# eric070021/TFHE-GPU

Measured on AMD Instinct MI355X. Metric: bootstraps/sec (whole node), STD128 GINX global batch=8192 (8192 per GPU, weak scaling), higher is better.
Workload: dtype u32; 1 GPU; C2: STD128 GINX EvalBinGate(NAND), inputs resident in HBM; config=C2, global_batch=8192, batch_per_gpu=8192, bootstraps_per_unit=1, n=512, N=1024, Q=134215681, dG2=8, parallelism=shard1

## Files before the change

tfhe-gpu_amd/csrc/blind_rotate_fast.hip:

```cpp
#include <atomic>
#include <cstdlib>

#include "device_math.hpp"
#include "kernels.hpp"

namespace tfhe {
namespace {

constexpr uint32_t FN = 1024;
constexpr uint32_t T4W = 5416, TB_WORDS = T4W;

struct FastConst {
    int32_t Q, nQ, qinv, rM;
    uint32_t Q2, Q4, h1, kacc;
    int32_t ninv;
    uint32_t bm;
};

struct PackMode {
    uint32_t hc[8];
    uint32_t rw;
    uint32_t fold;
};
__global__ void k_pack_fast(uint32_t Q, const uint32_t* __restrict__ bsk, size_t words, int32_t* __restrict__ out,
                            PackMode M) {
    const size_t idx = (size_t)blockIdx.x * blockDim.x + threadIdx.x;
    auto mont = [Q](uint32_t v) {
        const uint32_t m = (uint32_t)(((uint64_t)v << 32) % Q);
        return m > Q / 2 ? (int32_t)m - (int32_t)Q : (int32_t)m;
    };
    if (idx < words) {
        const uint32_t row = (uint32_t)((idx / (2 * FN)) % M.rw), l = row >> 1, p = row & 1, top = M.rw / 2 - 1;
        uint32_t v = bsk[idx] % Q;
// ... 10 lines not shown

static Fast4Shape fast_shape(const BRParams& P) {
    Fast4Shape sh{(int)P.digits, (int)P.logG, (int)P.thr, false};
    if (P.thr == 0 && P.digits >= 2 && P.logG >= 1 && P.logG * P.digits <= 40) {
        const int64_t G = (int64_t)1 << P.logG, Qh = (int64_t)(P.Q >> 1);
        const uint32_t top = P.digits - 1;
        int64_t K = 0;
        for (uint32_t z = 0; z < top; ++z) K = K * G + G / 2;
        const int64_t lo = (-Qh - 1 + K) >> (P.logG * top), hi = (Qh - 1 + K) >> (P.logG * top);
        sh.fold = lo >= -G / 2 && hi < G / 2;
    }
    return sh;
}

bool fast_path_supported(const BRParams& P, int word_bits) {
    return word_bits == 32 && P.N == FN && P.dG2 == 2 * P.digits && P.Q < (1ull << 27) && P.n > 0 &&
           fast4_shape_supported(fast_shape(P));
}

size_t bsk_fast_bytes(const BRParams& P) { return ((size_t)P.n * 2 * P.dG2 * 2 * FN + TB_WORDS) * 4; }

namespace {
constexpr int kDefaultVariant = 60;
bool known_variant(int v) { return v == 60 || v == 70 || v == 86; }
std::atomic<int> g_variant{-1};
int fast_variant() {
    int v = g_variant.load(std::memory_order_relaxed);
    if (v < 0) {
        const char* e = std::getenv("TFHE_FAST_VARIANT");
        v = e && e[0] ? std::atoi(e) : kDefaultVariant;
        if (!known_variant(v)) v = kDefaultVariant;
        g_variant.store(v, std::memory_order_relaxed);
    }
    return v;
}
uint64_t powmod(uint64_t b, uint64_t e, uint64_t m) {
    uint64_t r = 1 % m;
    for (b %= m; e; e >>= 1, b = (unsigned __int128)b * b % m)
        if (e & 1) r = (unsigned __int128)r * b % m;
    return r;
}
int32_t mont_centred(uint64_t v, uint32_t Q) {
    const uint32_t m = (uint32_t)(((unsigned __int128)(v % Q) << 32) % Q);
    return m > Q / 2 ? (int32_t)m - (int32_t)Q : (int32_t)m;
}
}

// ... 61 lines not shown
```

tfhe-gpu_amd/csrc/blind_rotate_fast4.hip:

```cpp
#include "device_math.hpp"
#include "kernels.hpp"

namespace tfhe {
namespace f4 {

constexpr uint32_t FN = 1024;
constexpr int TPC = 256;

constexpr uint32_t P0F = 0, P1F = 4, P2F = 20, P3F = 84, P4F = 340, PF_END = 1364;
constexpr uint32_t P0I = PF_END, P1I = P0I + P1F, P4I = P0I + P4F;
constexpr uint32_t T4_MONO = 2 * PF_END, T4_T1 = T4_MONO + 2 * FN, T4_T23 = T4_T1 + 128, T4_T2131 = T4_T23 + 256,
                   T4_WORDS = T4_T2131 + 256;
constexpr uint32_t L_TW = 0, L_TWI = P4F - P1F, L_MONO = 2 * L_TWI;
constexpr uint32_t L_T1 = L_MONO + 2 * FN, L_T23 = L_T1 + 128, L_T2131 = L_T23 + 256, L_P4F = L_T2131 + 256;
constexpr uint32_t LP = 304, XP = 1152, L_CT = L_P4F + 4 * 256;
constexpr uint32_t lds_ct(bool P4 = true) { return P4 ? L_CT : L_P4F; }
constexpr size_t lds_bytes(int P, int XB = 2, int CTS = 1, bool P4 = true) {
    return (size_t)(lds_ct(P4) + CTS * (4 * P * LP + XB * P * XP)) * 4;
}
constexpr bool pair_build(int MINW, int NCT, int OPT) { return MINW == 3 && NCT == 2 && (OPT & 8) == 0; }

struct Lay {
    int reg[2];
    int lane[6];
    int wave[2];
};
__host__ __device__ constexpr Lay lay(int L) {
    return L == 1   ? Lay{{8, 9}, {2, 3, 4, 6, 7, 5}, {0, 1}}
           : L == 2 ? Lay{{6, 7}, {2, 3, 8, 9, 4, 5}, {0, 1}}
           : L == 3 ? Lay{{4, 5}, {2, 3, 6, 8, 9, 7}, {0, 1}}
           : L == 4 ? Lay{{2, 3}, {4, 5, 6, 8, 9, 7}, {0, 1}}
                    : Lay{{0, 1}, {2, 3, 4, 5, 6, 7}, {8, 9}};
}
__host__ __device__ constexpr int rstride(int A, int B) {
    return (A == 1 && B == 2) ? 72 : (A == 2 && B == 3) ? 80 : (A == 3 && B == 4) ? 65
         : (A == 2 && B == 1) ? 68 : (A == 3 && B == 2) ? 68 : (A == 4 && B == 3) ? 65
// ... 75 lines not shown
__device__ __forceinline__ void bfly_ct(int32_t& a, int32_t& b, int32_t w, const FastConst& K) {
    const int32_t v = smul(b, w, K), u = a;
    a = u + v;
    b = u - v;
}
template <bool RED = false>
__device__ __forceinline__ void bfly_gs(int32_t& a, int32_t& b, int32_t w, const FastConst& K) {
    const int32_t u = a, v = b;
    a = RED ? smul(u + v, K.rM, K) : u + v;
    b = smul(u - v, w, K);
}
__device__ __forceinline__ void fwd4(int32_t (&x)[4], int32_t w1, int32_t w2, int32_t w3, const FastConst& K) {
    bfly_ct(x[0], x[2], w1, K);
    bfly_ct(x[1], x[3], w1, K);
    bfly_ct(x[0], x[1], w2, K);
    bfly_ct(x[2], x[3], w3, K);
}
template <bool RED>
__device__ __forceinline__ void inv4(int32_t (&x)[4], int32_t w1, int32_t w2, int32_t w3, const FastConst& K) {
    bfly_gs(x[0], x[1], w2, K);
    bfly_gs(x[2], x[3], w3, K);
    bfly_gs<RED>(x[0], x[2], w1, K);
    bfly_gs<RED>(x[1], x[3], w1, K);
}

template <int A, int B, uint32_t OFF>
__device__ __forceinline__ void store_rows(const int32_t (&x)[4], uint32_t m0, const int32_t* lds) {
    asm volatile(
        "s_mov_b32 m0, %4\n\t"
        "s_nop 0\n\t"
        "ds_write_addtid_b32 %0 offset:%6\n\t"
        "ds_write_addtid_b32 %1 offset:%7\n\t"
        "ds_write_addtid_b32 %2 offset:%8\n\t"
        "ds_write_addtid_b32 %3 offset:%9" ::"v"(x[0]),
        "v"(x[1]), "v"(x[2]), "v"(x[3]), "s"(m0), "s"(lds), "i"((OFF + st_reg(A, B, 0)) * 4),
        "i"((OFF + st_reg(A, B, 1)) * 4), "i"((OFF + st_reg(A, B, 2)) * 4), "i"((OFF + st_reg(A, B, 3)) * 4)
        : "memory");
}
template <int A, int B, uint32_t OFF>
__device__ __forceinline__ void gather_rows(int32_t (&x)[4], uint32_t base, const int32_t* lds) {
    asm volatile(
        "ds_read_b32 %0, %4 offset:%6\n\t"
        "ds_read_b32 %1, %4 offset:%7\n\t"
        "ds_read_b32 %2, %4 offset:%8\n\t"
        "ds_read_b32 %3, %4 offset:%9"
        : "=&v"(x[0]), "=&v"(x[1]), "=&v"(x[2]), "=&v"(x[3])
        : "v"(base), "s"(lds), "i"((OFF + ld_reg(A, B, 0)) * 4), "i"((OFF + ld_reg(A, B, 1)) * 4),
          "i"((OFF + ld_reg(A, B, 2)) * 4), "i"((OFF + ld_reg(A, B, 3)) * 4)
        : "memory");
}
template <uint32_t OFF>
__device__ __forceinline__ void tw_load(v4i& w, uint32_t addr, const int32_t* lds) {
    asm volatile("ds_read_b128 %0, %1 offset:%3" : "=&v"(w) : "v"(addr), "s"(lds), "i"(OFF * 4) : "memory");
}
template <int N>
__device__ __forceinline__ void lds_wait(int32_t (&x)[4]) {
    asm volatile("s_waitcnt lgkmcnt(%4)" : "+v"(x[0]), "+v"(x[1]), "+v"(x[2]), "+v"(x[3]) : "i"(N) : "memory");
}
template <int N>
__device__ __forceinline__ void lds_wait(int32_t (&x)[4], v4i& w) {
    asm volatile("s_waitcnt lgkmcnt(%5)"
                 : "+v"(x[0]), "+v"(x[1]), "+v"(x[2]), "+v"(x[3]), "+v"(w)
                 : "i"(N)
                 : "memory");
}
__device__ __forceinline__ void lds_drain_barrier() {
    asm volatile("s_waitcnt lgkmcnt(0)" ::: "memory");
    __syncthreads();
}

struct LaneCtx {
    uint32_t g12, g23, g34, g45, g54, g43, g32, g21;
    uint32_t m_loc;
    uint32_t m45, m54;
    uint32_t t1, t2, t3, t4;
    int32_t w0f[3], w0i[3];
    v4i w4f, w4i;
};

#define FOR_P(...)                                   \
    {                                                \
        { constexpr int p = 0; __VA_ARGS__ }         \
        if constexpr (P > 1) {                       \
            { constexpr int p = 1; __VA_ARGS__ }     \
        }                                            \
        if constexpr (P > 2) {                       \
            { constexpr int p = 2; __VA_ARGS__ }     \
            { constexpr int p = 3; __VA_ARGS__ }     \
        }                                            \
    }
template <int P, int p>
constexpr int tail_wait() { return 4 * (P - 1 - p); }

template <uint32_t XA, int P, int EXP = 0, int SMALL = 0, bool PRE = false, bool P4L = false>
__device__ __forceinline__ void ntt_fwd(int32_t (&X)[P][4], const int32_t* lds, const LaneCtx& C, const FastConst& K) {
    if constexpr ((EXP & 8) != 0) return;
    constexpr int W = 4 * (P - 1);
    v4i w;
    if constexpr (SMALL == 2) {
        const int32_t* t1 = lds + L_T1 + 64;
        const int2* t23 = reinterpret_cast<const int2*>(lds + L_T23) + 64;
        const int2* t2131 = reinterpret_cast<const int2*>(lds + L_T2131) + 64;
        int32_t a[P];
        int2 u23[P], u2131[P];
        FOR_P(a[p] = t1[X[p][2]]; u23[p] = t23[X[p][1]]; u2131[p] = t2131[X[p][3]];)
        FOR_P(const int32_t x0 = X[p][0], u = u23[p].x + u2131[p].x, v = u23[p].y - u2131[p].y;
              const int32_t e0 = x0 + a[p], e2 = x0 - a[p];
              X[p][0] = e0 + u; X[p][1] = e0 - u; X[p][2] = e2 + v; X[p][3] = e2 - v;
              store_rows<1, 2, p * LP>(X[p], C.m_loc, lds);)
    } else if constexpr (SMALL == 1) {
        const int32_t* t1 = lds + L_T1 + 64;
        int32_t v[P][2];
        FOR_P(v[p][0] = t1[X[p][2]]; v[p][1] = t1[X[p][3]];)
        FOR_P(const int32_t a0 = X[p][0], a1 = X[p][1];
              X[p][0] = a0 + v[p][0]; X[p][2] = a0 - v[p][0]; X[p][1] = a1 + v[p][1]; X[p][3] = a1 - v[p][1];
              bfly_ct(X[p][0], X[p][1], C.w0f[1], K); bfly_ct(X[p][2], X[p][3], C.w0f[2], K);
              store_rows<1, 2, p * LP>(X[p], C.m_loc, lds);)
    } else {
        FOR_P(fwd4(X[p], C.w0f[0], C.w0f[1], C.w0f[2], K); store_rows<1, 2, p * LP>(X[p], C.m_loc, lds);)
    }
    tw_load<L_TW>(w, C.t1, lds);
    FOR_P(gather_rows<1, 2, p * LP>(X[p], C.g12, lds);)
    FOR_P(if constexpr (p == 0) lds_wait<W>(X[0], w); else lds_wait<W>(X[p]);
          fwd4(X[p], w.x, w.y, w.z, K); store_rows<2, 3, p * LP>(X[p], C.m_loc, lds);)
    tw_load<L_TW + 16>(w, C.t2, lds);
    FOR_P(gather_rows<2, 3, p * LP>(X[p], C.g23, lds);)
    FOR_P(if constexpr (p == 0) lds_wait<W>(X[0], w); else lds_wait<W>(X[p]);
          fwd4(X[p], w.x, w.y, w.z, K); store_rows<3, 4, p * LP>(X[p], C.m_loc, lds);)
    tw_load<L_TW + 80>(w, C.t3, lds);
    FOR_P(gather_rows<3, 4, p * LP>(X[p], C.g34, lds);)
    FOR_P(if constexpr (p == 0) lds_wait<W>(X[0], w); else lds_wait<W>(X[p]);
          fwd4(X[p], w.x, w.y, w.z, K);
          if constexpr (PRE && p == 0) __builtin_amdgcn_s_barrier();
          store_rows<4, 5, XA + p * XP>(X[p], C.m45, lds);)
    if constexpr (!(EXP & 1)) lds_drain_barrier();
    if constexpr (P4L) tw_load<L_P4F>(w, C.t4, lds);
    FOR_P(gather_rows<4, 5, XA + p * XP>(X[p], C.g45, lds);)
    if constexpr (P4L) {
        FOR_P(if constexpr (p == 0) lds_wait<tail_wait<P, 0>()>(X[0], w); else lds_wait<tail_wait<P, p>()>(X[p]);
              fwd4(X[p], w.x, w.y, w.z, K);)
    } else {
        FOR_P(lds_wait<tail_wait<P, p>()>(X[p]); fwd4(X[p], C.w4f.x, C.w4f.y, C.w4f.z, K);)
    }
}

template <uint32_t XA, int P, int EXP = 0, bool PRE = false>
__device__ __forceinline__ void ntt_inv(int32_t (&X)[P][4], const int32_t* lds, const LaneCtx& C, const FastConst& K) {
    if constexpr ((EXP & 8) != 0) return;
    constexpr int W = 4 * (P - 1);
    v4i w;
    FOR_P(inv4<false>(X[p], C.w4i.x, C.w4i.y, C.w4i.z, K); if constexpr (PRE && p == 0) __builtin_amdgcn_s_barrier();
          store_rows<5, 4, XA + p * XP>(X[p], C.m54, lds);)
    if constexpr (!(EXP & 1)) lds_drain_barrier();
    tw_load<L_TWI + 80>(w, C.t3, lds);
    FOR_P(gather_rows<5, 4, XA + p * XP>(X[p], C.g54, lds);)
    FOR_P(if constexpr (p == 0) lds_wait<W>(X[0], w); else lds_wait<W>(X[p]);
          inv4<true>(X[p], w.x, w.y, w.z, K);
          store_rows<4, 3, p * LP>(X[p], C.m_loc, lds);)
    tw_load<L_TWI + 16>(w, C.t2, lds);
    FOR_P(gather_rows<4, 3, p * LP>(X[p], C.g43, lds);)
    FOR_P(if constexpr (p == 0) lds_wait<W>(X[0], w); else lds_wait<W>(X[p]);
          inv4<false>(X[p], w.x, w.y, w.z, K); store_rows<3, 2, p * LP>(X[p], C.m_loc, lds);)
    tw_load<L_TWI>(w, C.t1, lds);
    FOR_P(gather_rows<3, 2, p * LP>(X[p], C.g32, lds);)
    FOR_P(if constexpr (p == 0) lds_wait<W>(X[0], w); else lds_wait<W>(X[p]);
          inv4<true>(X[p], w.x, w.y, w.z, K); store_rows<2, 1, p * LP>(X[p], C.m_loc, lds);)
    FOR_P(gather_rows<2, 1, p * LP>(X[p], C.g21, lds);)
    FOR_P(lds_wait<tail_wait<P, p>()>(X[p]); inv4<false>(X[p], C.w0i[0], C.w0i[1], C.w0i[2], K);)
}

template <int MINW, int NCT = 1, int EXP = 0, int OPT = 7, int XB = 2, int CTS = 1, int DIG = 4, int LOGG = 7,
          int THR = 0, bool FOLD = true, bool FLAG = false, bool SPLIT = false, int RING = 4>
__global__ void __launch_bounds__(TPC * (SPLIT ? 2 : CTS), MINW)
k_blind_rotate_fast4(FastConst K, uint32_t n, uint32_t loga, const int32_t* __restrict__ tabs,
                     const int32_t* __restrict__ bsk, const uint64_t* __restrict__ a, uint64_t* __restrict__ acc_io,
                     uint32_t B, uint32_t* __restrict__ done) {
    constexpr int NPOL = SPLIT ? 1 : 2;
    constexpr int P = NPOL * NCT;
    constexpr int GR = SPLIT ? 2 : CTS;
    extern __shared__ __align__(16) int32_t lds[];
    static_assert(CTS == 1 || NCT == 1, "CTS > 1 needs NCT = 1");
    static_assert(RING == 4 || RING == 2, "key ring of four groups or two");
    constexpr uint32_t LCT = lds_ct(!pair_build(MINW, NCT, OPT));
    static_assert(!SPLIT || (NCT == 1 && CTS == 1 && FOLD && !FLAG && XB == 1), "SPLIT: the folded one-ciphertext build");
    constexpr uint32_t RW = 2 * DIG;
    constexpr int TOP = DIG - 1;
    constexpr int NT = FOLD ? DIG - 1 : DIG;
    static_assert(!FOLD || THR == 0, "top-digit elimination needs every digit");
    static_assert(LOGG * (THR + NT) <= 32, "digit field beyond 32 bits");
    static_assert(XB == 1 || (DIG == 4 && FOLD), "two cross areas need the STD128 digit order");
    const uint32_t cl = __builtin_amdgcn_readfirstlane(threadIdx.x / TPC);
    const uint32_t tid = threadIdx.x % TPC;
    const uint32_t wg_ct = SPLIT ? blockIdx.x : blockIdx.x * CTS * NCT + cl;
    const uint32_t pol = SPLIT ? cl : 0;
    for (uint32_t k = threadIdx.x; k < L_TWI; k += TPC * GR) lds[L_TW + k] = tabs[P1F + k], lds[L_TWI + k] = tabs[P1I + k];
    for (uint32_t k = threadIdx.x; k < 2 * FN + 640; k += TPC * GR) lds[L_MONO + k] = tabs[T4_MONO + k];
    if constexpr ((OPT & 8) != 0)
        for (uint32_t k = threadIdx.x; k < 4 * 256; k += TPC * GR) lds[L_P4F + k] = tabs[P4F + k];
    const uint32_t w = __builtin_amdgcn_readfirstlane(tid >> 6), lane = tid & 63;
    constexpr uint32_t LOCW = P * LP, XAW = P * XP;
    constexpr uint32_t XA0 = 4 * LOCW, XA1 = XB == 2 ? XA0 + XAW : XA0;
    constexpr bool PRE = XB == 1;

    LaneCtx C;
    constexpr uint32_t CTW = 4 * LOCW + XB * XAW;
    const uint32_t ctb = (LCT + cl * CTW) * 4;
    C.m_loc = ctb + w * LOCW * 4;
    C.g12 = C.m_loc + ld_lane<1, 2>(w, lane) * 4, C.g23 = C.m_loc + ld_lane<2, 3>(w, lane) * 4;
    C.g34 = C.m_loc + ld_lane<3, 4>(w, lane) * 4, C.g43 = C.m_loc + ld_lane<4, 3>(w, lane) * 4;
    C.g32 = C.m_loc + ld_lane<3, 2>(w, lane) * 4, C.g21 = C.m_loc + ld_lane<2, 1>(w, lane) * 4;
    C.g45 = ctb + ld_lane<4, 5>(w, lane) * 4, C.g54 = ctb + ld_lane<5, 4>(w, lane) * 4;
    C.m45 = ctb + st_wave<4, 5>(w) * 4, C.m54 = ctb + st_wave<5, 4>(w) * 4;
    C.t1 = (elem<2>(w, lane, 0) >> 8) * 16, C.t2 = (elem<3>(w, lane, 0) >> 6) * 16;
    C.t3 = (elem<4>(w, lane, 0) >> 4) * 16, C.t4 = tid * 16;
    const v4i* tv = reinterpret_cast<const v4i*>(tabs);
    if constexpr ((OPT & 8) == 0) C.w4f = tv[P4F / 4 + tid];
    C.w4i = tv[P4I / 4 + tid];
#pragma unroll
    for (int k = 0; k < 3; ++k) C.w0f[k] = tabs[P0F + k], C.w0i[k] = tabs[P0I + k];

    const uint32_t Qh = (uint32_t)K.Q >> 1;
    int32_t acc[NCT][NPOL][4];
#pragma unroll
    for (int q = 0; q < NCT; ++q) {
        const uint32_t ct = wg_ct + q;
        const uint64_t* g = acc_io + (size_t)(ct < B ? ct : 0) * 2 * FN;
#pragma unroll
        for (int p = 0; p < NPOL; ++p)
#pragma unroll
            for (int r = 0; r < 4; ++r) {
                const uint64_t v0 = ct < B ? g[(SPLIT ? pol : p) * FN + elem<1>(w, lane, r)] : 0;
                const uint32_t v = (uint32_t)(v0 >= (uint64_t)K.Q ? v0 % (uint64_t)K.Q : v0);
                acc[q][p][r] = v < Qh ? (int32_t)v : (int32_t)v - K.Q;
            }
    }
    __syncthreads();

    int32_t Cp[P][4];
    if constexpr (FOLD) {
        if constexpr (SPLIT) {
#pragma unroll
            for (int r = 0; r < 4; ++r) Cp[0][r] = acc[0][0][r];
        } else {
#pragma unroll
            for (int q = 0; q < NCT; ++q)
#pragma unroll
                for (int r = 0; r < 4; ++r) Cp[2 * q][r] = acc[q][0][r], Cp[2 * q + 1][r] = acc[q][NPOL - 1][r];
        }
        ntt_fwd<XA1, P, EXP, 0, PRE, (OPT & 8) != 0>(Cp, lds, C, K);
#pragma unroll
        for (int p = 0; p < P; ++p)
#pragma unroll
            for (int r = 0; r < 4; ++r) Cp[p][r] = smul(Cp[p][r], K.ninv, K);
    }

    constexpr uint32_t ROWB = 2 * RW * 2 * FN * 4;
    const __amdgpu_buffer_rsrc_t rsrc =
        __builtin_amdgcn_make_buffer_rsrc(const_cast<int32_t*>(bsk), 0, (int)(n * ROWB), 0x00020000);
    const uint32_t voff = tid * 16;
    const uint32_t et = 2 * (__builtin_bitreverse32(tid) >> 24) + 1;
    const uint32_t amask = (1u << loga) - 1, ashift = 11 - loga;

    auto issue = [&](v4i (&pw)[2], uint32_t round_off, int l, int gi) {
        const int k = gi >> 1, j = gi & 1;
        if constexpr ((EXP & 2) != 0) {
            pw[0] = v4i{(int)round_off, l, gi, 4}, pw[1] = pw[0] + 1;
            return;
        }
        if constexpr (SPLIT) {
            pw[0] = ld_bsk(rsrc, voff, round_off + ((k * RW + 2 * l + pol) * 2 + j) * FN * 4);
            return;
        }
        pw[0] = ld_bsk(rsrc, voff, round_off + ((k * RW + 2 * l) * 2 + j) * FN * 4);
        pw[1] = ld_bsk(rsrc, voff, round_off + ((k * RW + 2 * l + 1) * 2 + j) * FN * 4);
    };
    auto mac = [&](int64_t (&s)[NCT][2][2][4], const int32_t (&X)[P][4], const v4i (&pw)[2], int gi, bool first) {
        const int k = gi >> 1, j = gi & 1;
        const int32_t w0[4] = {pw[0].x, pw[0].y, pw[0].z, pw[0].w};
        const int32_t w1[4] = {pw[1].x, pw[1].y, pw[1].z, pw[1].w};
#pragma unroll
        for (int q = 0; q < NCT; ++q)
#pragma unroll
            for (int r = 0; r < 4; ++r) {
// ... 42 lines not shown
        } else {
#pragma unroll
            for (int gi = 0; gi < RING; ++gi) issue(pw[gi], round_off, 0, gi);
        }
#pragma unroll
        for (uint32_t l = 0; l < NT; ++l) {
            const uint32_t lt = l + THR;
            const int32_t kl = (int32_t)(((1u << (LOGG * lt)) - 1) / ((1u << LOGG) - 1)) << (LOGG - 1);
            int32_t X[P][4];
            if constexpr (SPLIT) {
#pragma unroll
                for (int r = 0; r < 4; ++r) X[0][r] = __builtin_amdgcn_sbfe(acc[0][0][r] + kl, LOGG * lt, LOGG);
            } else {
#pragma unroll
                for (int q = 0; q < NCT; ++q)
#pragma unroll
                    for (int r = 0; r < 4; ++r) {
                        X[2 * q][r] = __builtin_amdgcn_sbfe(acc[q][0][r] + kl, LOGG * lt, LOGG);
                        X[2 * q + 1][r] = __builtin_amdgcn_sbfe(acc[q][NPOL - 1][r] + kl, LOGG * lt, LOGG);
                    }
            }
            __builtin_amdgcn_sched_barrier(0);
            constexpr int SM = LOGG > 7 ? 0 : (OPT & 4) ? 2 : (OPT & 1) ? 1 : 0;
            if (l & 1) ntt_fwd<XA1, P, EXP, SM, PRE, (OPT & 8) != 0>(X, lds, C, K);
            else ntt_fwd<XA0, P, EXP, SM, PRE, (OPT & 8) != 0>(X, lds, C, K);
            const bool last = l + 1 == NT;
            const uint32_t noff = !last ? round_off : (i + 1 < n ? i + 1 : i) * ROWB;
            const int nl = !last ? (int)l + 1 : TOP;
#pragma unroll
            for (int gi = 0; gi < 4; ++gi) {
                __builtin_amdgcn_sched_barrier(0);
                mac(s, X, pw[gi % RING], gi, !FOLD && l == 0);
                if constexpr (RING == 4) {
                    if (FOLD || !last) issue(pw[gi], noff, nl, gi);
                } else {
                    step2(round_off, (int)l, noff, nl, gi, !last);
                }
            }
        }

        __builtin_amdgcn_sched_barrier(0);
        const char* mono = reinterpret_cast<const char*>(lds + L_MONO);
        int32_t S[P][4];
        if constexpr (SPLIT) {
            int32_t* xch = lds + LCT + GR * (4 * P * LP + XB * P * XP);
            const uint32_t bp = (et * ai[0]) & 2047, bn = (0u - bp) & 2047;
            const uint32_t F4p = ((bp >> 4) & 0x1C) | ((bp & 63) << 7), F4n = ((bn >> 4) & 0x1C) | ((bn & 63) << 7);
            const uint32_t hp = (bp >> 4) & 0x60, hn = (bn >> 4) & 0x60;
            int32_t Am[2][4];
#pragma unroll
            for (int k = 0; k < 2; ++k)
#pragma unroll
                for (int r = 0; r < 4; ++r) {
                    xch[((pol * 2 + k) * 4 + r) * TPC + tid] = sredc(pol ? s[0][k][0][r] : s[0][k][1][r], K);
                    Am[k][r] = sredc(pol ? s[0][k][1][r] : s[0][k][0][r], K);
                }
            __syncthreads();
#pragma unroll
            for (int r = 0; r < 4; ++r) {
                const uint32_t c = ((r & 1) << 1) | (r >> 1);
                const uint32_t cs = c * 32 * ai[0];
                const int32_t mp = *reinterpret_cast<const int32_t*>(mono + ((((hp + cs) & 0x60)) | F4p));
                const int32_t mn = *reinterpret_cast<const int32_t*>(mono + ((((hn - cs) & 0x60)) | F4n));
                const int32_t A0 = Am[0][r] + xch[(((1 - pol) * 2 + 0) * 4 + r) * TPC + tid];
// ... 16 lines not shown
                const int32_t A10 = sredc(s[q][1][0][r], K), A11 = sredc(s[q][1][1][r], K);
                S[2 * q][r] = sredc((int64_t)A00 * mp + (int64_t)A10 * mn, K);
                S[2 * q + 1][r] = sredc((int64_t)A01 * mp + (int64_t)A11 * mn, K);
            }
        }
        if constexpr (FOLD) {
#pragma unroll
            for (int p = 0; p < P; ++p)
#pragma unroll
                for (int r = 0; r < 4; ++r) Cp[p][r] += S[p][r];
        }
        if (FOLD && (i & 7) == 7) {
#pragma unroll
            for (int p = 0; p < P; ++p)
#pragma unroll
                for (int r = 0; r < 4; ++r) Cp[p][r] = smul(Cp[p][r], K.rM, K);
        }
        __builtin_amdgcn_sched_barrier(0);
        if constexpr (FOLD && RING == 2) {
            const uint32_t noff = (i + 1 < n ? i + 1 : i) * ROWB;
            issue(pw[0], noff, TOP, 0), issue(pw[1], noff, TOP, 1);
            __builtin_amdgcn_sched_barrier(0);
        }
        ntt_inv<XA1, P, EXP, PRE>(S, lds, C, K);
#pragma unroll
        for (int q = 0; q < NCT; ++q)
#pragma unroll
            for (int p = 0; p < NPOL; ++p)
#pragma unroll
                for (int r = 0; r < 4; ++r) {
                    uint32_t u = (uint32_t)(acc[q][p][r] + S[NPOL * q + p][r]) + K.kacc;
                    if constexpr ((OPT & 2) != 0) {
                        const uint32_t qt = __umulhi(u, K.bm);
                        uint64_t t;
                        asm("v_mad_u64_u32 %0, vcc, %1, %2, %3" : "=v"(t) : "v"(qt), "s"(K.nQ), "v"((uint64_t)u) : "vcc");
                        u = csub32((uint32_t)t, (uint32_t)K.Q);
                    } else {
                        u = csub32(csub32(csub32(u, K.Q4), K.Q2), (uint32_t)K.Q);
                    }
                    acc[q][p][r] = (int32_t)(u - K.h1);
                }
    }
#pragma unroll
    for (int q = 0; q < NCT; ++q) {
        const uint32_t ct = wg_ct + q;
        if (ct >= B) continue;
        uint64_t* g = acc_io + (size_t)ct * 2 * FN;
// ... 31 lines not shown
        if (idx < P1F) m = 1, base = P0F;
        else if (idx < P2F) m = 4, base = P1F;
        else if (idx < P3F) m = 16, base = P2F;
        else if (idx < P4F) m = 64, base = P3F;
        else m = 256, base = P4F;
        const uint32_t c = (idx - base) >> 2, e = (idx - base) & 3;
        const uint32_t k = e == 0 ? m + c : 2 * m + 2 * c + (e - 1);
        out[idx] = e == 3 ? 0 : mont(psi[k]);
        out[P0I + idx] = e == 3 ? 0 : mont(ipsi[k]);
    }
    if (idx < 2 * FN) out[T4_MONO + ((idx >> 6) | ((idx & 63) << 5))] = mont(mono[idx]);
    if (idx < 128) {
        const int32_t d = (int32_t)idx - 64;
        auto dmul = [Q, d](uint64_t w) {
            const uint32_t v = (uint32_t)((uint64_t)(uint32_t)(d < 0 ? -d : d) * (w % Q) % Q);
            const uint32_t m = d < 0 ? (v ? Q - v : 0) : v;
            return m > Q / 2 ? (int32_t)m - (int32_t)Q : (int32_t)m;
        };
        const uint64_t p21 = (uint64_t)psi[2] * psi[1] % Q, p31 = (uint64_t)psi[3] * psi[1] % Q;
        out[T4_T1 + idx] = dmul(psi[1]);
        out[T4_T23 + 2 * idx] = dmul(psi[2]), out[T4_T23 + 2 * idx + 1] = dmul(psi[3]);
        out[T4_T2131 + 2 * idx] = dmul(p21), out[T4_T2131 + 2 * idx + 1] = dmul(p31);
    }
}

#endif
}
#ifndef TFHE_FAST4_KERNEL_ONLY

size_t fast4_table_words() { return f4::T4_WORDS; }
size_t fast4_lds_bytes(bool pair) { return pair ? f4::lds_bytes(4, 1, 1, false) : f4::lds_bytes(2, 1, 1); }

hipError_t launch_pack_tables_fast4(uint32_t Q, const DevTables& T, void* out, hipStream_t s) {
    hipLaunchKernelGGL(f4::k_pack_tables4, dim3((f4::T4_WORDS + 255) / 256), dim3(256), 0, s, Q,
                       (const uint32_t*)T.psi, (const uint32_t*)T.ipsi, (const uint32_t*)T.mono, (int32_t*)out);
    return hipGetLastError();
}

bool fast4_shape_supported(const Fast4Shape& sh) {
    return (sh.dig == 4 && sh.logg == 7 && sh.thr == 0 && sh.fold) ||
           (sh.dig == 6 && sh.logg == 5 && sh.thr == 0 && sh.fold) ||
           (sh.dig == 5 && sh.logg == 5 && sh.thr == 1 && !sh.fold) ||
           (sh.dig == 3 && sh.logg == 9 && sh.thr == 0 && !sh.fold);
}

hipError_t launch_blind_rotate_fast4_d6(const f4::FastConst& K, uint32_t n, uint32_t loga, const int32_t* tabs4,
                                        const int32_t* bsk, const uint64_t* a, uint64_t* acc, size_t B, hipStream_t s);

hipError_t launch_blind_rotate_fast4_pair(const f4::FastConst& K, uint32_t n, uint32_t loga, const int32_t* tabs4,
                                          const int32_t* bsk, const uint64_t* a, uint64_t* acc, size_t B, hipStream_t s);

hipError_t launch_blind_rotate_fast4(int variant, const Fast4Shape& sh, const void* K, uint32_t n, uint32_t loga,
                                     const int32_t* tabs4, const int32_t* bsk, const uint64_t* a, uint64_t* acc,
                                     size_t B, hipStream_t s, BRDone* dn, int split_max, int pair_min, bool* paired) {
    const f4::FastConst Kc = *reinterpret_cast<const f4::FastConst*>(K);
    auto launch = [&](auto kern, int nct, int xb = 2, int cts = 1, uint32_t* done = nullptr) {
        const size_t lb = f4::lds_bytes(2 * nct, xb, cts);
        (void)hipFuncSetAttribute((const void*)kern, hipFuncAttributeMaxDynamicSharedMemorySize, (int)lb);
        hipLaunchKernelGGL(kern, dim3((unsigned)((B + nct * cts - 1) / (nct * cts))), dim3(f4::TPC * cts), lb, s, Kc,
                           n, loga, tabs4, bsk, a, acc, (uint32_t)B, done);
    };
    if (sh.dig == 6 && sh.logg == 5 && sh.thr == 0 && sh.fold)
        return launch_blind_rotate_fast4_d6(Kc, n, loga, tabs4, bsk, a, acc, B, s);
    if (sh.dig == 5 && sh.logg == 5 && sh.thr == 1 && !sh.fold) {
        launch(f4::k_blind_rotate_fast4<4, 1, 0, 7, 1, 1, 5, 5, 1, false>, 1, 1);
        return hipGetLastError();
    }
    if (sh.dig == 3 && sh.logg == 9 && sh.thr == 0 && !sh.fold) {
        launch(f4::k_blind_rotate_fast4<4, 1, 0, 7, 1, 1, 3, 9, 0, false>, 1, 1);
        return hipGetLastError();
    }
    if (!(sh.dig == 4 && sh.logg == 7 && sh.thr == 0 && sh.fold)) return hipErrorNotSupported;
    if (variant == 60 && B <= (size_t)split_max && !(dn && dn->flags)) {
        auto kern = f4::k_blind_rotate_fast4<4, 1, 0, 7, 1, 1, 4, 7, 0, true, false, true>;
        const size_t lb = f4::lds_bytes(1, 1, 2) + (size_t)2 * 8 * f4::TPC * 4;
        (void)hipFuncSetAttribute((const void*)kern, hipFuncAttributeMaxDynamicSharedMemorySize, (int)lb);
        hipLaunchKernelGGL(kern, dim3((unsigned)B), dim3(2 * f4::TPC), lb, s, Kc, n, loga, tabs4, bsk, a, acc, (uint32_t)B,
                           (uint32_t*)nullptr);
        return hipGetLastError();
    }
    if (dn && dn->flags && variant == 60) {
        launch(f4::k_blind_rotate_fast4<4, 1, 0, 7, 1, 1, 4, 7, 0, true, true>, 1, 1, 1, dn->flags);
        dn->written = true;
        return hipGetLastError();
    }
    if (variant == 70 || (variant == 60 && pair_min > 0 && B >= (size_t)pair_min)) {
        if (paired) *paired = true;
        return launch_blind_rotate_fast4_pair(Kc, n, loga, tabs4, bsk, a, acc, B, s);
    }
    switch (variant) {
        case 86: launch(f4::k_blind_rotate_fast4<4, 1, 0, 7, 1, 4>, 1, 1, 4); break;
        default: launch(f4::k_blind_rotate_fast4<4, 1, 0, 7, 1>, 1, 1); break;
    }
    return hipGetLastError();
}

#endif
}

#if defined(TFHE_TEST_PROBES) && !defined(TFHE_FAST4_KERNEL_ONLY)
#include "arith_probes.hpp"

namespace tfhe {
namespace f4 {
constexpr int F4P_NI = 8, F4P_NO = 4;
__global__ void k_arith_fast4(int op, size_t cases, const uint64_t* __restrict__ in, const uint64_t* __restrict__,
                              size_t, uint64_t* __restrict__ out, FastConst K) {
    const size_t i = (size_t)blockIdx.x * blockDim.x + threadIdx.x;
    if (!probe_lane_runs(op, i, cases)) return;
    const int64_t* x = reinterpret_cast<const int64_t*>(in) + i * F4P_NI;
    int64_t* o = reinterpret_cast<int64_t*>(out) + i * F4P_NO;
    const int f = op & 15;
    if (f == 0) o[0] = sredc(x[0], K);
    else if (f == 1) o[0] = smul((int32_t)x[0], (int32_t)x[1], K);
    else if (f == 2) o[0] = (int64_t)(uint64_t)csub32((uint32_t)x[0], (uint32_t)x[1]);
    else if (f >= 3 && f <= 5) {
        int32_t a = (int32_t)x[0], b = (int32_t)x[1];
        if (f == 3) bfly_ct(a, b, (int32_t)x[2], K);
        else if (f == 4) bfly_gs<false>(a, b, (int32_t)x[2], K);
        else bfly_gs<true>(a, b, (int32_t)x[2], K);
        o[0] = a, o[1] = b;
    } else if (f >= 6 && f <= 8) {
        int32_t v[4] = {(int32_t)x[0], (int32_t)x[1], (int32_t)x[2], (int32_t)x[3]};
        const int32_t w1 = (int32_t)x[4], w2 = (int32_t)x[5], w3 = (int32_t)x[6];
        if (f == 6) fwd4(v, w1, w2, w3, K);
        else if (f == 7) inv4<false>(v, w1, w2, w3, K);
        else inv4<true>(v, w1, w2, w3, K);
#pragma unroll
        for (int k = 0; k < 4; ++k) o[k] = v[k];
    }
}
}
}

extern "C" TFHE_ARITH_PROBE(fast4) {
    if ((op & 15) > 8 || Q < 3 || Q >= (1ull << 27) || !(Q & 1)) return -1;
    tfhe::f4::FastConst K;
    tfhe::fast_const_build((uint32_t)Q, &K);
    return tfhe::probe_launch(tfhe::f4::k_arith_fast4, tfhe::f4::F4P_NI, tfhe::f4::F4P_NO, op, cases, in, in_words, tab,
                              tab_words, out, out_words, K);
}
#endif
```

tfhe-gpu_amd/csrc/blind_rotate_fast4_pair.hip:

```cpp
#define TFHE_FAST4_KERNEL_ONLY
#include "blind_rotate_fast4.hip"

namespace tfhe {

hipError_t launch_blind_rotate_fast4_pair(const f4::FastConst& K, uint32_t n, uint32_t loga, const int32_t* tabs4,
                                          const int32_t* bsk, const uint64_t* a, uint64_t* acc, size_t B, hipStream_t s) {
    auto kern = f4::k_blind_rotate_fast4<3, 2, 0, 7, 1, 1, 4, 7, 0, true, false, false, 2>;
    const size_t lb = f4::lds_bytes(4, 1, 1, false);
    (void)hipFuncSetAttribute((const void*)kern, hipFuncAttributeMaxDynamicSharedMemorySize, (int)lb);
    hipLaunchKernelGGL(kern, dim3((unsigned)((B + 1) / 2)), dim3(f4::TPC), lb, s, K, n, loga, tabs4, bsk, a, acc,
                       (uint32_t)B, nullptr);
    return hipGetLastError();
}

}
```

Baseline: 200,900 bootstraps/s.

## Fuse radix-4 NTT butterflies with precombined twiddle products in paired blind-rotate kernel

Adds fused radix-4 forward and inverse butterflies that fold two twiddle multiplies into a single 64-bit multiply-accumulate and one Montgomery reduction, using precomputed products of twiddle pairs. It also stores a single mirrored twiddle table in LDS that serves both the forward and inverse passes, instead of two separate tables. The aim is fewer modular reductions and less LDS footprint and loading per NTT pass. In exchange it adds extra LDS reads for the side twiddle, a larger packed table, and new kernel variants. It is enabled by default only on the paired path (variant 60 with pair_min, or variant 70/71).

Measured after the change: 210,200 bootstraps/s, median of 6. +4.6%, better.

```diff
diff --git a/tfhe-gpu_amd/csrc/blind_rotate_fast.hip b/tfhe-gpu_amd/csrc/blind_rotate_fast.hip
--- a/tfhe-gpu_amd/csrc/blind_rotate_fast.hip
+++ b/tfhe-gpu_amd/csrc/blind_rotate_fast.hip
@@ -8,7 +8,7 @@
 namespace {
 
 constexpr uint32_t FN = 1024;
-constexpr uint32_t T4W = 5416, TB_WORDS = T4W;
+constexpr uint32_t T4W = 6864, TB_WORDS = T4W;
 
 struct FastConst {
     int32_t Q, nQ, qinv, rM;
@@ -65,7 +65,7 @@
 
 namespace {
 constexpr int kDefaultVariant = 60;
-bool known_variant(int v) { return v == 60 || v == 70 || v == 86; }
+bool known_variant(int v) { return v == 60 || v == 61 || v == 70 || v == 71 || v == 86; }
 std::atomic<int> g_variant{-1};
 int fast_variant() {
     int v = g_variant.load(std::memory_order_relaxed);
diff --git a/tfhe-gpu_amd/csrc/blind_rotate_fast4.hip b/tfhe-gpu_amd/csrc/blind_rotate_fast4.hip
--- a/tfhe-gpu_amd/csrc/blind_rotate_fast4.hip
+++ b/tfhe-gpu_amd/csrc/blind_rotate_fast4.hip
@@ -9,9 +9,13 @@
 
 constexpr uint32_t P0F = 0, P1F = 4, P2F = 20, P3F = 84, P4F = 340, PF_END = 1364;
 constexpr uint32_t P0I = PF_END, P1I = P0I + P1F, P4I = P0I + P4F;
-constexpr uint32_t T4_MONO = 2 * PF_END, T4_T1 = T4_MONO + 2 * FN, T4_T23 = T4_T1 + 128, T4_T2131 = T4_T23 + 256,
-                   T4_WORDS = T4_T2131 + 256;
+constexpr uint32_t T4_MONO = 2 * PF_END, T4_T1 = T4_MONO + 2 * FN, T4_T23 = T4_T1 + 128, T4_T2131 = T4_T23 + 256;
+constexpr uint32_t FUL_BLK = P4F - P1F, FUL_WORDS = FUL_BLK + FUL_BLK / 4;
+constexpr uint32_t T4_FU0 = T4_T2131 + 256, T4_FUL = T4_FU0 + 4, T4_FU4 = T4_FUL + FUL_WORDS, T4_WORDS = T4_FU4 + 4 * 256;
+enum : int { FU_F0 = 1, FU_L = 2, FU_F4 = 4, FU_I5 = 8, FU_I1 = 16, FU_LF = 32, FU_ALL = 63 };
 constexpr uint32_t L_TW = 0, L_TWI = P4F - P1F, L_MONO = 2 * L_TWI;
+constexpr uint32_t L_N31 = L_TW + FUL_BLK;
+static_assert(FUL_WORDS <= L_MONO, "the shared table fits the two tables' area");
 constexpr uint32_t L_T1 = L_MONO + 2 * FN, L_T23 = L_T1 + 128, L_T2131 = L_T23 + 256, L_P4F = L_T2131 + 256;
 constexpr uint32_t LP = 304, XP = 1152, L_CT = L_P4F + 4 * 256;
 constexpr uint32_t lds_ct(bool P4 = true) { return P4 ? L_CT : L_P4F; }
@@ -133,6 +137,24 @@
     bfly_gs(x[2], x[3], w3, K);
     bfly_gs<RED>(x[0], x[2], w1, K);
     bfly_gs<RED>(x[1], x[3], w1, K);
+}
+
+__device__ __forceinline__ void fwd4f(int32_t (&x)[4], int32_t w1, int32_t w2, int32_t w3, int32_t p21, int32_t n31,
+                                      const FastConst& K) {
+    const int32_t t = smul(x[2], w1, K), a = x[0] + t, b = x[0] - t;
+    const int32_t c = sredc(mac64(x[3], p21, (int64_t)x[1] * w2), K);
+    const int32_t d = sredc(mac64(x[3], n31, (int64_t)x[1] * w3), K);
+    x[0] = a + c, x[1] = a - c, x[2] = b + d, x[3] = b - d;
+}
+template <bool RED, bool MIR>
+__device__ __forceinline__ void inv4f(int32_t (&x)[4], int32_t w1, int32_t wa, int32_t wb, int32_t pa, int32_t pb,
+                                      const FastConst& K) {
+    const int32_t e = MIR ? x[1] - x[0] : x[0] - x[1], f = MIR ? x[3] - x[2] : x[2] - x[3];
+    const int32_t s0 = x[0] + x[1], s2 = x[2] + x[3];
+    x[1] = sredc(mac64(f, wb, (int64_t)e * wa), K);
+    x[3] = sredc(mac64(f, pb, (int64_t)e * pa), K);
+    x[2] = smul(MIR ? s2 - s0 : s0 - s2, w1, K);
+    x[0] = RED ? smul(s0 + s2, K.rM, K) : s0 + s2;
 }
 
 template <int A, int B, uint32_t OFF>
@@ -164,6 +186,28 @@
 __device__ __forceinline__ void tw_load(v4i& w, uint32_t addr, const int32_t* lds) {
     asm volatile("ds_read_b128 %0, %1 offset:%3" : "=&v"(w) : "v"(addr), "s"(lds), "i"(OFF * 4) : "memory");
 }
+template <uint32_t OFF>
+__device__ __forceinline__ void tw_load1(int32_t& w, uint32_t addr, const int32_t* lds) {
+    asm volatile("ds_read_b32 %0, %1 offset:%3" : "=&v"(w) : "v"(addr), "s"(lds), "i"(OFF * 4) : "memory");
+}
+template <uint32_t M>
+__device__ __forceinline__ uint32_t tw_mirror(uint32_t t) {
+    uint32_t r;
+    asm volatile("v_sub_u32_e32 %0, %1, %2" : "=v"(r) : "i"((M - 1) * 16), "v"(t));
+    return r;
+}
+__device__ __forceinline__ uint32_t tw_side(uint32_t t) {
+    uint32_t r;
+    asm volatile("v_lshrrev_b32_e32 %0, 2, %1" : "=v"(r) : "v"(t));
+    return r;
+}
+template <int N>
+__device__ __forceinline__ void lds_wait(int32_t (&x)[4], v4i& w, int32_t& w5) {
+    asm volatile("s_waitcnt lgkmcnt(%6)"
+                 : "+v"(x[0]), "+v"(x[1]), "+v"(x[2]), "+v"(x[3]), "+v"(w), "+v"(w5)
+                 : "i"(N)
+                 : "memory");
+}
 template <int N>
 __device__ __forceinline__ void lds_wait(int32_t (&x)[4]) {
     asm volatile("s_waitcnt lgkmcnt(%4)" : "+v"(x[0]), "+v"(x[1]), "+v"(x[2]), "+v"(x[3]) : "i"(N) : "memory");
@@ -187,6 +231,8 @@
     uint32_t t1, t2, t3, t4;
     int32_t w0f[3], w0i[3];
     v4i w4f, w4i;
+    int32_t p0f[2], p0i[2];
+    int32_t x4f, x4i;
 };
 
 #define FOR_P(...)                                   \
@@ -203,11 +249,25 @@
 template <int P, int p>
 constexpr int tail_wait() { return 4 * (P - 1 - p); }
 
-template <uint32_t XA, int P, int EXP = 0, int SMALL = 0, bool PRE = false, bool P4L = false>
+template <uint32_t XA, int P, int EXP = 0, int SMALL = 0, bool PRE = false, bool P4L = false, int FU = 0>
 __device__ __forceinline__ void ntt_fwd(int32_t (&X)[P][4], const int32_t* lds, const LaneCtx& C, const FastConst& K) {
     if constexpr ((EXP & 8) != 0) return;
     constexpr int W = 4 * (P - 1);
+    static_assert(!(P4L && (FU & FU_F4)), "fused pass 4 takes its twiddles from registers");
+    static_assert(!(FU & FU_LF) || (FU & FU_L), "fused forward passes 1-3 need the shared table");
     v4i w;
+    int32_t w5 = 0;
+#define TW_LOAD(OFF, T)                                                  \
+    tw_load<L_TW + OFF>(w, T, lds);                                      \
+    if constexpr ((FU & FU_LF) != 0) tw_load1<L_N31 + OFF / 4>(w5, tw_side(T), lds);
+#define FWD_PASS(p)                                                                         \
+    if constexpr ((FU & FU_LF) != 0) {                                                      \
+        if constexpr (p == 0) lds_wait<W>(X[0], w, w5); else lds_wait<W>(X[p]);             \
+        fwd4f(X[p], w.x, w.y, w.z, w.w, w5, K);                                             \
+    } else {                                                                                \
+        if constexpr (p == 0) lds_wait<W>(X[0], w); else lds_wait<W>(X[p]);                 \
+        fwd4(X[p], w.x, w.y, w.z, K);                                                       \
+    }
     if constexpr (SMALL == 2) {
         const int32_t* t1 = lds + L_T1 + 64;
         const int2* t23 = reinterpret_cast<const int2*>(lds + L_T23) + 64;
@@ -227,21 +287,20 @@
               X[p][0] = a0 + v[p][0]; X[p][2] = a0 - v[p][0]; X[p][1] = a1 + v[p][1]; X[p][3] = a1 - v[p][1];
               bfly_ct(X[p][0], X[p][1], C.w0f[1], K); bfly_ct(X[p][2], X[p][3], C.w0f[2], K);
               store_rows<1, 2, p * LP>(X[p], C.m_loc, lds);)
+    } else if constexpr ((FU & FU_F0) != 0) {
+        FOR_P(fwd4f(X[p], C.w0f[0], C.w0f[1], C.w0f[2], C.p0f[0], C.p0f[1], K); store_rows<1, 2, p * LP>(X[p], C.m_loc, lds);)
     } else {
         FOR_P(fwd4(X[p], C.w0f[0], C.w0f[1], C.w0f[2], K); store_rows<1, 2, p * LP>(X[p], C.m_loc, lds);)
     }
-    tw_load<L_TW>(w, C.t1, lds);
+    TW_LOAD(0, C.t1)
     FOR_P(gather_rows<1, 2, p * LP>(X[p], C.g12, lds);)
-    FOR_P(if constexpr (p == 0) lds_wait<W>(X[0], w); else lds_wait<W>(X[p]);
-          fwd4(X[p], w.x, w.y, w.z, K); store_rows<2, 3, p * LP>(X[p], C.m_loc, lds);)
-    tw_load<L_TW + 16>(w, C.t2, lds);
+    FOR_P(FWD_PASS(p) store_rows<2, 3, p * LP>(X[p], C.m_loc, lds);)
+    TW_LOAD(16, C.t2)
     FOR_P(gather_rows<2, 3, p * LP>(X[p], C.g23, lds);)
-    FOR_P(if constexpr (p == 0) lds_wait<W>(X[0], w); else lds_wait<W>(X[p]);
-          fwd4(X[p], w.x, w.y, w.z, K); store_rows<3, 4, p * LP>(X[p], C.m_loc, lds);)
-    tw_load<L_TW + 80>(w, C.t3, lds);
+    FOR_P(FWD_PASS(p) store_rows<3, 4, p * LP>(X[p], C.m_loc, lds);)
+    TW_LOAD(80, C.t3)
     FOR_P(gather_rows<3, 4, p * LP>(X[p], C.g34, lds);)
-    FOR_P(if constexpr (p == 0) lds_wait<W>(X[0], w); else lds_wait<W>(X[p]);
-          fwd4(X[p], w.x, w.y, w.z, K);
+    FOR_P(FWD_PASS(p)
           if constexpr (PRE && p == 0) __builtin_amdgcn_s_barrier();
           store_rows<4, 5, XA + p * XP>(X[p], C.m45, lds);)
     if constexpr (!(EXP & 1)) lds_drain_barrier();
@@ -250,38 +309,62 @@
     if constexpr (P4L) {
         FOR_P(if constexpr (p == 0) lds_wait<tail_wait<P, 0>()>(X[0], w); else lds_wait<tail_wait<P, p>()>(X[p]);
               fwd4(X[p], w.x, w.y, w.z, K);)
+    } else if constexpr ((FU & FU_F4) != 0) {
+        FOR_P(lds_wait<tail_wait<P, p>()>(X[p]);
+              fwd4f(X[p], C.w4f.x, C.w4f.y, C.w4f.z, C.w4f.w, (FU & FU_I5) ? C.x4f : C.w4i.w, K);)
     } else {
         FOR_P(lds_wait<tail_wait<P, p>()>(X[p]); fwd4(X[p], C.w4f.x, C.w4f.y, C.w4f.z, K);)
     }
-}
-
-template <uint32_t XA, int P, int EXP = 0, bool PRE = false>
+#undef TW_LOAD
+#undef FWD_PASS
+}
+
+template <uint32_t XA, int P, int EXP = 0, bool PRE = false, int FU = 0>
 __device__ __forceinline__ void ntt_inv(int32_t (&X)[P][4], const int32_t* lds, const LaneCtx& C, const FastConst& K) {
     if constexpr ((EXP & 8) != 0) return;
     constexpr int W = 4 * (P - 1);
     v4i w;
-    FOR_P(inv4<false>(X[p], C.w4i.x, C.w4i.y, C.w4i.z, K); if constexpr (PRE && p == 0) __builtin_amdgcn_s_barrier();
+    int32_t w5 = 0;
+#define TWI_LOAD(OFF, M, T)                                                  \
+    if constexpr ((FU & FU_L) != 0) {                                        \
+        const uint32_t tm = tw_mirror<M>(T);                                 \
+        tw_load<L_TW + OFF>(w, tm, lds);                                     \
+        tw_load1<L_N31 + OFF / 4>(w5, tw_side(tm), lds);                     \
+    } else {                                                                 \
+        tw_load<L_TWI + OFF>(w, T, lds);                                     \
+    }
+#define INV_PASS(p, RED)                                                                    \
+    if constexpr ((FU & FU_L) != 0) {                                                       \
+        if constexpr (p == 0) lds_wait<W>(X[0], w, w5); else lds_wait<W>(X[p]);             \
+        inv4f<RED, true>(X[p], w.x, w.z, w.y, w5, w.w, K);                                  \
+    } else {                                                                                \
+        if constexpr (p == 0) lds_wait<W>(X[0], w); else lds_wait<W>(X[p]);                 \
+        inv4<RED>(X[p], w.x, w.y, w.z, K);                                                  \
+    }
+    FOR_P(if constexpr ((FU & FU_I5) != 0) inv4f<false, false>(X[p], C.w4i.x, C.w4i.y, C.w4i.z, C.w4i.w, C.x4i, K);
+          else inv4<false>(X[p], C.w4i.x, C.w4i.y, C.w4i.z, K);
+          if constexpr (PRE && p == 0) __builtin_amdgcn_s_barrier();
           store_rows<5, 4, XA + p * XP>(X[p], C.m54, lds);)
     if constexpr (!(EXP & 1)) lds_drain_barrier();
-    tw_load<L_TWI + 80>(w, C.t3, lds);
+    TWI_LOAD(80, 64, C.t3)
     FOR_P(gather_rows<5, 4, XA + p * XP>(X[p], C.g54, lds);)
-    FOR_P(if constexpr (p == 0) lds_wait<W>(X[0], w); else lds_wait<W>(X[p]);
-          inv4<true>(X[p], w.x, w.y, w.z, K);
-          store_rows<4, 3, p * LP>(X[p], C.m_loc, lds);)
-    tw_load<L_TWI + 16>(w, C.t2, lds);
+    FOR_P(INV_PASS(p, true) store_rows<4, 3, p * LP>(X[p], C.m_loc, lds);)
+    TWI_LOAD(16, 16, C.t2)
     FOR_P(gather_rows<4, 3, p * LP>(X[p], C.g43, lds);)
-    FOR_P(if constexpr (p == 0) lds_wait<W>(X[0], w); else lds_wait<W>(X[p]);
-          inv4<false>(X[p], w.x, w.y, w.z, K); store_rows<3, 2, p * LP>(X[p], C.m_loc, lds);)
-    tw_load<L_TWI>(w, C.t1, lds);
+    FOR_P(INV_PASS(p, false) store_rows<3, 2, p * LP>(X[p], C.m_loc, lds);)
+    TWI_LOAD(0, 4, C.t1)
     FOR_P(gather_rows<3, 2, p * LP>(X[p], C.g32, lds);)
-    FOR_P(if constexpr (p == 0) lds_wait<W>(X[0], w); else lds_wait<W>(X[p]);
-          inv4<true>(X[p], w.x, w.y, w.z, K); store_rows<2, 1, p * LP>(X[p], C.m_loc, lds);)
+    FOR_P(INV_PASS(p, true) store_rows<2, 1, p * LP>(X[p], C.m_loc, lds);)
     FOR_P(gather_rows<2, 1, p * LP>(X[p], C.g21, lds);)
-    FOR_P(lds_wait<tail_wait<P, p>()>(X[p]); inv4<false>(X[p], C.w0i[0], C.w0i[1], C.w0i[2], K);)
+    FOR_P(lds_wait<tail_wait<P, p>()>(X[p]);
+          if constexpr ((FU & FU_I1) != 0) inv4f<false, false>(X[p], C.w0i[0], C.w0i[1], C.w0i[2], C.p0i[0], C.p0i[1], K);
+          else inv4<false>(X[p], C.w0i[0], C.w0i[1], C.w0i[2], K);)
+#undef TWI_LOAD
+#undef INV_PASS
 }
 
 template <int MINW, int NCT = 1, int EXP = 0, int OPT = 7, int XB = 2, int CTS = 1, int DIG = 4, int LOGG = 7,
-          int THR = 0, bool FOLD = true, bool FLAG = false, bool SPLIT = false, int RING = 4>
+          int THR = 0, bool FOLD = true, bool FLAG = false, bool SPLIT = false, int RING = 4, int FU = 0>
 __global__ void __launch_bounds__(TPC * (SPLIT ? 2 : CTS), MINW)
 k_blind_rotate_fast4(FastConst K, uint32_t n, uint32_t loga, const int32_t* __restrict__ tabs,
                      const int32_t* __restrict__ bsk, const uint64_t* __restrict__ a, uint64_t* __restrict__ acc_io,
@@ -304,7 +387,12 @@
     const uint32_t tid = threadIdx.x % TPC;
     const uint32_t wg_ct = SPLIT ? blockIdx.x : blockIdx.x * CTS * NCT + cl;
     const uint32_t pol = SPLIT ? cl : 0;
-    for (uint32_t k = threadIdx.x; k < L_TWI; k += TPC * GR) lds[L_TW + k] = tabs[P1F + k], lds[L_TWI + k] = tabs[P1I + k];
+    static_assert(!(FU & (FU_F4 | FU_I5)) || (OPT & 8) == 0, "fused pass 4 takes its twiddles from registers");
+    if constexpr ((FU & FU_L) != 0) {
+        for (uint32_t k = threadIdx.x; k < FUL_WORDS; k += TPC * GR) lds[L_TW + k] = tabs[T4_FUL + k];
+    } else {
+        for (uint32_t k = threadIdx.x; k < L_TWI; k += TPC * GR) lds[L_TW + k] = tabs[P1F + k], lds[L_TWI + k] = tabs[P1I + k];
+    }
     for (uint32_t k = threadIdx.x; k < 2 * FN + 640; k += TPC * GR) lds[L_MONO + k] = tabs[T4_MONO + k];
     if constexpr ((OPT & 8) != 0)
         for (uint32_t k = threadIdx.x; k < 4 * 256; k += TPC * GR) lds[L_P4F + k] = tabs[P4F + k];
@@ -324,11 +412,22 @@
     C.m45 = ctb + st_wave<4, 5>(w) * 4, C.m54 = ctb + st_wave<5, 4>(w) * 4;
     C.t1 = (elem<2>(w, lane, 0) >> 8) * 16, C.t2 = (elem<3>(w, lane, 0) >> 6) * 16;
     C.t3 = (elem<4>(w, lane, 0) >> 4) * 16, C.t4 = tid * 16;
+    if constexpr ((FU & FU_L) != 0) C.t3 = lane * 16;
     const v4i* tv = reinterpret_cast<const v4i*>(tabs);
     if constexpr ((OPT & 8) == 0) C.w4f = tv[P4F / 4 + tid];
     C.w4i = tv[P4I / 4 + tid];
 #pragma unroll
     for (int k = 0; k < 3; ++k) C.w0f[k] = tabs[P0F + k], C.w0i[k] = tabs[P0I + k];
+    if constexpr ((FU & (FU_F0 | FU_I1)) != 0) {
+#pragma unroll
+        for (int k = 0; k < 2; ++k) C.p0f[k] = tabs[T4_FU0 + k], C.p0i[k] = tabs[T4_FU0 + 2 + k];
+    }
+    if constexpr ((FU & (FU_F4 | FU_I5)) != 0) {
+        const v4i x4 = tv[T4_FU4 / 4 + tid];
+        if constexpr ((FU & FU_F4) != 0) C.w4f.w = x4.x, C.x4f = x4.y;
+        if constexpr ((FU & FU_I5) != 0) C.w4i.w = x4.z, C.x4i = x4.w;
+        else C.w4i.w = x4.y;
+    }
 
     const uint32_t Qh = (uint32_t)K.Q >> 1;
     int32_t acc[NCT][NPOL][4];
@@ -358,7 +457,7 @@
 #pragma unroll
                 for (int r = 0; r < 4; ++r) Cp[2 * q][r] = acc[q][0][r], Cp[2 * q + 1][r] = acc[q][NPOL - 1][r];
         }
-        ntt_fwd<XA1, P, EXP, 0, PRE, (OPT & 8) != 0>(Cp, lds, C, K);
+        ntt_fwd<XA1, P, EXP, 0, PRE, (OPT & 8) != 0, FU>(Cp, lds, C, K);
 #pragma unroll
         for (int p = 0; p < P; ++p)
 #pragma unroll
@@ -369,7 +468,7 @@
     const __amdgpu_buffer_rsrc_t rsrc =
         __builtin_amdgcn_make_buffer_rsrc(const_cast<int32_t*>(bsk), 0, (int)(n * ROWB), 0x00020000);
     const uint32_t voff = tid * 16;
-    const uint32_t et = 2 * (__builtin_bitreverse32(tid) >> 24) + 1;
+    const uint32_t et0 = 2 * (__builtin_bitreverse32(tid) >> 24) + 1;
     const uint32_t amask = (1u << loga) - 1, ashift = 11 - loga;
 
     auto issue = [&](v4i (&pw)[2], uint32_t round_off, int l, int gi) {
@@ -458,8 +557,8 @@
             }
             __builtin_amdgcn_sched_barrier(0);
             constexpr int SM = LOGG > 7 ? 0 : (OPT & 4) ? 2 : (OPT & 1) ? 1 : 0;
-            if (l & 1) ntt_fwd<XA1, P, EXP, SM, PRE, (OPT & 8) != 0>(X, lds, C, K);
-            else ntt_fwd<XA0, P, EXP, SM, PRE, (OPT & 8) != 0>(X, lds, C, K);
+            if (l & 1) ntt_fwd<XA1, P, EXP, SM, PRE, (OPT & 8) != 0, FU>(X, lds, C, K);
+            else ntt_fwd<XA0, P, EXP, SM, PRE, (OPT & 8) != 0, FU>(X, lds, C, K);
             const bool last = l + 1 == NT;
             const uint32_t noff = !last ? round_off : (i + 1 < n ? i + 1 : i) * ROWB;
             const int nl = !last ? (int)l + 1 : TOP;
@@ -476,6 +575,12 @@
         }
 
         __builtin_amdgcn_sched_barrier(0);
+        uint32_t et = et0;
+        if constexpr ((FU & (FU_F4 | FU_I5)) != 0) {
+            uint32_t br;
+            asm volatile("v_bfrev_b32_e32 %0, %1" : "=v"(br) : "v"(voff));
+            et = ((br >> 19) & 0x1FE) | 1;
+        }
         const char* mono = reinterpret_cast<const char*>(lds + L_MONO);
         int32_t S[P][4];
         if constexpr (SPLIT) {
@@ -538,7 +643,7 @@
             issue(pw[0], noff, TOP, 0), issue(pw[1], noff, TOP, 1);
             __builtin_amdgcn_sched_barrier(0);
         }
-        ntt_inv<XA1, P, EXP, PRE>(S, lds, C, K);
+        ntt_inv<XA1, P, EXP, PRE, FU>(S, lds, C, K);
 #pragma unroll
         for (int q = 0; q < NCT; ++q)
 #pragma unroll
@@ -616,6 +721,20 @@
         out[T4_T23 + 2 * idx] = dmul(psi[2]), out[T4_T23 + 2 * idx + 1] = dmul(psi[3]);
         out[T4_T2131 + 2 * idx] = dmul(p21), out[T4_T2131 + 2 * idx + 1] = dmul(p31);
     }
+    auto pn = [Q, &mont](const uint32_t* t, uint32_t m, uint32_t c, bool neg) {
+        const uint32_t v = (uint32_t)((uint64_t)t[2 * m + 2 * c + (neg ? 1 : 0)] * t[m + c] % Q);
+        return mont(neg ? (v ? Q - v : 0) : v);
+    };
+    if (idx < FUL_BLK) {
+        const uint32_t m = idx < P2F - P1F ? 4 : idx < P3F - P1F ? 16 : 64, base = m == 4 ? 0 : m == 16 ? P2F - P1F : P3F - P1F;
+        uint32_t c = (idx - base) >> 2;
+        const uint32_t e = idx & 3;
+        if (m == 64) c = (c & 7) | ((c & 8) << 1) | ((c & 16) << 1) | ((c & 32) >> 2);
+        out[T4_FUL + idx] = e == 3 ? pn(psi, m, c, false) : mont(psi[e == 0 ? m + c : 2 * m + 2 * c + (e - 1)]);
+        if (e == 3) out[T4_FUL + FUL_BLK + (idx >> 2)] = pn(psi, m, c, true);
+    }
+    if (idx < 4) out[T4_FU0 + idx] = pn(idx < 2 ? psi : ipsi, 1, 0, idx & 1);
+    if (idx < 4 * 256) out[T4_FU4 + idx] = pn((idx & 2) ? ipsi : psi, 256, idx >> 2, idx & 1);
 }
 
 #endif
@@ -642,7 +761,10 @@
                                         const int32_t* bsk, const uint64_t* a, uint64_t* acc, size_t B, hipStream_t s);
 
 hipError_t launch_blind_rotate_fast4_pair(const f4::FastConst& K, uint32_t n, uint32_t loga, const int32_t* tabs4,
-                                          const int32_t* bsk, const uint64_t* a, uint64_t* acc, size_t B, hipStream_t s);
+                                          const int32_t* bsk, const uint64_t* a, uint64_t* acc, size_t B, hipStream_t s,
+                                          bool fused);
+
+constexpr bool kPairFused = true;
 
 hipError_t launch_blind_rotate_fast4(int variant, const Fast4Shape& sh, const void* K, uint32_t n, uint32_t loga,
                                      const int32_t* tabs4, const int32_t* bsk, const uint64_t* a, uint64_t* acc,
@@ -678,12 +800,16 @@
         dn->written = true;
         return hipGetLastError();
     }
-    if (variant == 70 || (variant == 60 && pair_min > 0 && B >= (size_t)pair_min)) {
+    if (variant == 70 || variant == 71 || (variant == 60 && pair_min > 0 && B >= (size_t)pair_min)) {
         if (paired) *paired = true;
-        return launch_blind_rotate_fast4_pair(Kc, n, loga, tabs4, bsk, a, acc, B, s);
+        return launch_blind_rotate_fast4_pair(Kc, n, loga, tabs4, bsk, a, acc, B, s,
+                                              variant == 60 ? kPairFused : variant == 71);
     }
     switch (variant) {
         case 86: launch(f4::k_blind_rotate_fast4<4, 1, 0, 7, 1, 4>, 1, 1, 4); break;
+        case 61:
+            launch(f4::k_blind_rotate_fast4<4, 1, 0, 7, 1, 1, 4, 7, 0, true, false, false, 4, f4::FU_F0 | f4::FU_L | f4::FU_I1>, 1, 1);
+            break;
         default: launch(f4::k_blind_rotate_fast4<4, 1, 0, 7, 1>, 1, 1); break;
     }
     return hipGetLastError();
@@ -697,14 +823,14 @@
 
 namespace tfhe {
 namespace f4 {
-constexpr int F4P_NI = 8, F4P_NO = 4;
+constexpr int F4P_NI = 8, F4P_NO = 4, F4P_NIF = 10;
 __global__ void k_arith_fast4(int op, size_t cases, const uint64_t* __restrict__ in, const uint64_t* __restrict__,
                               size_t, uint64_t* __restrict__ out, FastConst K) {
     const size_t i = (size_t)blockIdx.x * blockDim.x + threadIdx.x;
     if (!probe_lane_runs(op, i, cases)) return;
-    const int64_t* x = reinterpret_cast<const int64_t*>(in) + i * F4P_NI;
+    const int f = op & 15;
+    const int64_t* x = reinterpret_cast<const int64_t*>(in) + i * (f >= 9 ? F4P_NIF : F4P_NI);
     int64_t* o = reinterpret_cast<int64_t*>(out) + i * F4P_NO;
-    const int f = op & 15;
     if (f == 0) o[0] = sredc(x[0], K);
     else if (f == 1) o[0] = smul((int32_t)x[0], (int32_t)x[1], K);
     else if (f == 2) o[0] = (int64_t)(uint64_t)csub32((uint32_t)x[0], (uint32_t)x[1]);
@@ -722,16 +848,26 @@
         else inv4<true>(v, w1, w2, w3, K);
 #pragma unroll
         for (int k = 0; k < 4; ++k) o[k] = v[k];
+    } else if (f >= 9 && f <= 13) {
+        int32_t v[4] = {(int32_t)x[0], (int32_t)x[1], (int32_t)x[2], (int32_t)x[3]};
+        const int32_t w1 = (int32_t)x[4], w2 = (int32_t)x[5], w3 = (int32_t)x[6], pa = (int32_t)x[7], pb = (int32_t)x[8];
+        if (f == 9) fwd4f(v, w1, w2, w3, pa, pb, K);
+        else if (f == 10) inv4f<false, false>(v, w1, w2, w3, pa, pb, K);
+        else if (f == 11) inv4f<true, false>(v, w1, w2, w3, pa, pb, K);
+        else if (f == 12) inv4f<false, true>(v, w1, w2, w3, pa, pb, K);
+        else inv4f<true, true>(v, w1, w2, w3, pa, pb, K);
+#pragma unroll
+        for (int k = 0; k < 4; ++k) o[k] = v[k];
     }
 }
 }
 }
 
 extern "C" TFHE_ARITH_PROBE(fast4) {
-    if ((op & 15) > 8 || Q < 3 || Q >= (1ull << 27) || !(Q & 1)) return -1;
+    if ((op & 15) > 13 || Q < 3 || Q >= (1ull << 27) || !(Q & 1)) return -1;
     tfhe::f4::FastConst K;
     tfhe::fast_const_build((uint32_t)Q, &K);
-    return tfhe::probe_launch(tfhe::f4::k_arith_fast4, tfhe::f4::F4P_NI, tfhe::f4::F4P_NO, op, cases, in, in_words, tab,
+    return tfhe::probe_launch(tfhe::f4::k_arith_fast4, (op & 15) >= 9 ? tfhe::f4::F4P_NIF : tfhe::f4::F4P_NI, tfhe::f4::F4P_NO, op, cases, in, in_words, tab,
                               tab_words, out, out_words, K);
 }
 #endif
diff --git a/tfhe-gpu_amd/csrc/blind_rotate_fast4_pair.hip b/tfhe-gpu_amd/csrc/blind_rotate_fast4_pair.hip
--- a/tfhe-gpu_amd/csrc/blind_rotate_fast4_pair.hip
+++ b/tfhe-gpu_amd/csrc/blind_rotate_fast4_pair.hip
@@ -3,9 +3,16 @@
 
 namespace tfhe {
 
+#ifndef TFHE_PAIR_FU
+#define TFHE_PAIR_FU (f4::FU_ALL & ~f4::FU_F4)
+#endif
+constexpr int PAIR_FU = TFHE_PAIR_FU;
+
 hipError_t launch_blind_rotate_fast4_pair(const f4::FastConst& K, uint32_t n, uint32_t loga, const int32_t* tabs4,
-                                          const int32_t* bsk, const uint64_t* a, uint64_t* acc, size_t B, hipStream_t s) {
-    auto kern = f4::k_blind_rotate_fast4<3, 2, 0, 7, 1, 1, 4, 7, 0, true, false, false, 2>;
+                                          const int32_t* bsk, const uint64_t* a, uint64_t* acc, size_t B, hipStream_t s,
+                                          bool fused) {
+    auto kern = fused ? f4::k_blind_rotate_fast4<3, 2, 0, 7, 1, 1, 4, 7, 0, true, false, false, 2, PAIR_FU>
+                      : f4::k_blind_rotate_fast4<3, 2, 0, 7, 1, 1, 4, 7, 0, true, false, false, 2>;
     const size_t lb = f4::lds_bytes(4, 1, 1, false);
     (void)hipFuncSetAttribute((const void*)kern, hipFuncAttributeMaxDynamicSharedMemorySize, (int)lb);
     hipLaunchKernelGGL(kern, dim3((unsigned)((B + 1) / 2)), dim3(f4::TPC), lb, s, K, n, loga, tabs4, bsk, a, acc,
```
